# marja-w/gan-des-midi-music-gen

Measured on AMD Instinct MI355X. Metric: GAN training samples/sec (G+D step), higher is better.
Workload: dtype bf16; 1 GPU; SIMNN G/D iteration, synthetic 128x256 spectrogram windows; per_gpu_batch=256, global_batch=256, mode=faithful, parallelism=dp1

## Files before the change

### gan_des_midi_music_gen_amd/csrc/gemm.hip

```cpp
#include "gemm_common.h"

namespace {

constexpr int BM = 64, BN = 64, NT = 256;

template <typename CT> struct GemmCfg;
template <> struct GemmCfg<float> { static constexpr int KT = 32, LD = 34; };
template <> struct GemmCfg<__bf16> { static constexpr int KT = 64, LD = 72; };

template <typename CT, typename TA, typename TB>
__global__ __launch_bounds__(NT) void gemm_kernel(GemmArgs g) {
  constexpr int KT = GemmCfg<CT>::KT, LD = GemmCfg<CT>::LD;
  __shared__ __attribute__((aligned(16))) CT smem[(BM + BN) * LD];
  CT* As = smem;
  CT* Bs = smem + BM * LD;
  const int t = threadIdx.x, l = t & 63, w = t >> 6, wm = w >> 1, wn = w & 1;
  const int lr = l & 15, lg = l >> 4;
  const int m0 = blockIdx.y * BM, n0 = blockIdx.x * BN;
  const int kbeg = blockIdx.z * g.k_per_split;
  const int kend = min(g.K, kbeg + g.k_per_split);
  const TA* __restrict__ A = (const TA*)g.A;
  const TB* __restrict__ B = (const TB*)g.B;
  const bool a_kfast = (g.sak == 1), b_kfast = (g.sbk == 1);
  f32x4 acc[2][2];
#pragma unroll
  for (int i = 0; i < 2; ++i)
#pragma unroll
    for (int j = 0; j < 2; ++j) acc[i][j] = (f32x4){0.f, 0.f, 0.f, 0.f};

  constexpr int PER = BM * KT / NT;
  float va[PER], vb[PER];
  auto load_tile = [&](int k0) {
#pragma unroll
    for (int i = 0; i < PER; ++i) {
      const int idx = t + NT * i;
      const int m = a_kfast ? idx / KT : idx % BM;
      const int k = a_kfast ? idx % KT : idx / BM;
      const int gm = m0 + m, gk = k0 + k;
      va[i] = (gm < g.M && gk < kend) ? to_f32(A[(int64_t)gm * g.sam + (int64_t)gk * g.sak]) : 0.f;
    }
#pragma unroll
    for (int i = 0; i < PER; ++i) {
      const int idx = t + NT * i;
      const int n = b_kfast ? idx / KT : idx % BN;
      const int k = b_kfast ? idx % KT : idx / BN;
      const int gn = n0 + n, gk = k0 + k;
      vb[i] = (gn < g.N && gk < kend) ? to_f32(B[(int64_t)gk * g.sbk + (int64_t)gn * g.sbn]) : 0.f;
    }
  };
  if (kbeg < kend) load_tile(kbeg);
  for (int k0 = kbeg; k0 < kend; k0 += KT) {
#pragma unroll
    for (int i = 0; i < PER; ++i) {
      const int idx = t + NT * i;
      const int m = a_kfast ? idx / KT : idx % BM;
      const int k = a_kfast ? idx % KT : idx / BM;
      As[m * LD + k] = from_f32<CT>(va[i]);
      const int n = b_kfast ? idx / KT : idx % BN;
      const int kb = b_kfast ? idx % KT : idx / BN;
      Bs[n * LD + kb] = from_f32<CT>(vb[i]);
    }
    __syncthreads();
    if (k0 + KT < kend) load_tile(k0 + KT);
    if constexpr (sizeof(CT) == 4) {
#pragma unroll
      for (int ks = 0; ks < KT / 4; ++ks) {
        float a[2], b[2];
#pragma unroll
        for (int i = 0; i < 2; ++i) a[i] = As[(wm * 32 + i * 16 + lr) * LD + ks * 4 + lg];
#pragma unroll
        for (int j = 0; j < 2; ++j) b[j] = Bs[(wn * 32 + j * 16 + lr) * LD + ks * 4 + lg];
#pragma unroll
        for (int i = 0; i < 2; ++i)
#pragma unroll
          for (int j = 0; j < 2; ++j) acc[i][j] = mfma16(a[i], b[j], acc[i][j]);
      }
    } else {
#pragma unroll
      for (int ks = 0; ks < KT / 32; ++ks) {
        bf16x8 a[2], b[2];
#pragma unroll
        for (int i = 0; i < 2; ++i) a[i] = *(const bf16x8*)&As[(wm * 32 + i * 16 + lr) * LD + ks * 32 + lg * 8];
#pragma unroll
        for (int j = 0; j < 2; ++j) b[j] = *(const bf16x8*)&Bs[(wn * 32 + j * 16 + lr) * LD + ks * 32 + lg * 8];
#pragma unroll
        for (int i = 0; i < 2; ++i)
#pragma unroll
          for (int j = 0; j < 2; ++j) acc[i][j] = mfma16(a[i], b[j], acc[i][j]);
      }
    }
    __syncthreads();
  }

#pragma unroll
  for (int i = 0; i < 2; ++i)
#pragma unroll
    for (int j = 0; j < 2; ++j)
#pragma unroll
      for (int r = 0; r < 4; ++r) {
        const int m = m0 + wm * 32 + i * 16 + lg * 4 + r;
        const int n = n0 + wn * 32 + j * 16 + lr;
        if (m < g.M && n < g.N) {
          if (g.split_k > 1) g.ws[((int64_t)blockIdx.z * g.M + m) * g.N + n] = acc[i][j][r];
          else gemm_epilogue_store(g, m, n, acc[i][j][r]);
        }
      }
}

template <bool VEC>
__global__ __launch_bounds__(256) void gemm_splitk_reduce(GemmArgs g) {
  const int64_t total = (int64_t)g.M * g.N;
  if constexpr (VEC) {
    __shared__ f32x4 part[4][64];
    const int lane = threadIdx.x & 63, zg = threadIdx.x >> 6;
    const int64_t idx = ((int64_t)blockIdx.x * 64 + lane) * 4;
    const bool live = idx < total;
    const int q4 = (g.split_k + 3) / 4;
    const int z0 = zg * q4, z1 = min(g.split_k, z0 + q4);
    f32x4 s[4];
#pragma unroll
    for (int q = 0; q < 4; ++q) s[q] = (f32x4){0.f, 0.f, 0.f, 0.f};
    if (live) {
      int z = z0;
      for (; z + 3 < z1; z += 4) {
#pragma unroll
        for (int q = 0; q < 4; ++q) s[q] += *(const f32x4*)(g.ws + (int64_t)(z + q) * total + idx);
      }
      for (; z < z1; ++z) s[0] += *(const f32x4*)(g.ws + (int64_t)z * total + idx);
    }
    part[zg][lane] = (s[0] + s[1]) + (s[2] + s[3]);
    __syncthreads();
    if (zg == 0 && live) {
      const f32x4 v = (part[0][lane] + part[1][lane]) + (part[2][lane] + part[3][lane]);
      const int m = (int)(idx / g.N), n = (int)(idx % g.N);
#pragma unroll
      for (int r = 0; r < 4; ++r) gemm_epilogue_store(g, m, n + r, v[r]);
    }
  } else {
    const int64_t idx = (int64_t)blockIdx.x * 256 + threadIdx.x;
    if (idx >= total) return;
    float s[4] = {0.f, 0.f, 0.f, 0.f};
    int z = 0;
    for (; z + 3 < g.split_k; z += 4) {
#pragma unroll
      for (int q = 0; q < 4; ++q) s[q] += g.ws[(int64_t)(z + q) * total + idx];
    }
    for (; z < g.split_k; ++z) s[0] += g.ws[(int64_t)z * total + idx];
    gemm_epilogue_store(g, (int)(idx / g.N), (int)(idx % g.N), (s[0] + s[1]) + (s[2] + s[3]));
  }
}

int launch_splitk_reduce(const GemmArgs& g, hipStream_t s) {
  if (g.split_k > 1) {
    const int64_t total = (int64_t)g.M * g.N;
    if (g.N % 4 == 0) {
      hipLaunchKernelGGL(gemm_splitk_reduce<true>, dim3((unsigned)((total / 4 + 63) / 64)), dim3(256), 0, s, g);
    } else {
      hipLaunchKernelGGL(gemm_splitk_reduce<false>, dim3((unsigned)((total + 255) / 256)), dim3(256), 0, s, g);
    }
    GDM_LAUNCH_OK("gdm_gemm(split-k reduce)");
  }
  return GDM_OK;
}

template <typename CT>
int launch_gemm(const GemmArgs& g, int a_dtype, int b_dtype, hipStream_t s) {
  dim3 grid((g.N + BN - 1) / BN, (g.M + BM - 1) / BM, g.split_k), block(NT);
  if (a_dtype == GDM_F32 && b_dtype == GDM_F32) hipLaunchKernelGGL((gemm_kernel<CT, float, float>), grid, block, 0, s, g);
  else if (a_dtype == GDM_F32) hipLaunchKernelGGL((gemm_kernel<CT, float, __bf16>), grid, block, 0, s, g);
  else if (b_dtype == GDM_F32) hipLaunchKernelGGL((gemm_kernel<CT, __bf16, float>), grid, block, 0, s, g);
  else hipLaunchKernelGGL((gemm_kernel<CT, __bf16, __bf16>), grid, block, 0, s, g);
  GDM_LAUNCH_OK("gdm_gemm");
  return launch_splitk_reduce(g, s);
}

}

extern "C" int gdm_gemm(const void* A, int a_dtype, int64_t sam, int64_t sak, const void* B, int b_dtype, int64_t sbk,
                        int64_t sbn, void* C, int c_dtype, int64_t scm, int64_t scn, int M, int N, int K,
                        const float* bias_n, const float* bias_m, int act, float slope, int compute_dtype, int split_k,
                        void* workspace, size_t workspace_bytes, void* stream) {
  GDM_REQUIRE(A && B && C, "gdm_gemm: null operand");
  GDM_REQUIRE(M > 0 && N > 0 && K > 0, "gdm_gemm: bad dims M=%d N=%d K=%d", M, N, K);
  GDM_REQUIRE(gdm_dtype_ok(a_dtype) && gdm_dtype_ok(b_dtype) && gdm_dtype_ok(c_dtype) && gdm_dtype_ok(compute_dtype),
              "gdm_gemm: bad dtype");
  GDM_REQUIRE(act >= GDM_ACT_NONE && act <= GDM_ACT_SIGMOID, "gdm_gemm: bad activation %d", act);
  GDM_REQUIRE(split_k >= 1 && split_k <= 65535, "gdm_gemm: bad split_k %d", split_k);
  GemmArgs probe{A, sam, sak, B, sbk, sbn, C, c_dtype, scm, scn, M, N, K, bias_n, bias_m, act, slope, 1, K, nullptr};
  const bool fast = compute_dtype == GDM_BF16 && gdm_gemm_bf16_fast_ok(probe, a_dtype, b_dtype);
  const int KT = fast ? GDM_GEMM_FAST_KT : (compute_dtype == GDM_BF16 ? GemmCfg<__bf16>::KT : GemmCfg<float>::KT);
  int tiles = (K + KT - 1) / KT;
  if (split_k > tiles) split_k = tiles;
  int per = (tiles + split_k - 1) / split_k;
  split_k = (tiles + per - 1) / per;
  if (split_k > 1) {
    if (workspace == nullptr || workspace_bytes < (size_t)split_k * M * N * sizeof(float)) {
      gdm_set_error("gdm_gemm: split_k=%d needs %zu workspace bytes, got %zu", split_k,
                    (size_t)split_k * M * N * sizeof(float), workspace_bytes);
      return GDM_EWORKSPACE;
    }
  }
  GemmArgs g{A, sam, sak, B, sbk, sbn, C, c_dtype, scm, scn, M, N, K, bias_n, bias_m, act, slope,
             split_k, per * KT, (float*)workspace};
  hipStream_t s = (hipStream_t)stream;
  if (fast) {
    int rc = gdm_gemm_bf16_fast_launch(g, a_dtype, b_dtype, s);
    if (rc != GDM_OK) return rc;
    return launch_splitk_reduce(g, s);
  }
  return compute_dtype == GDM_BF16 ? launch_gemm<__bf16>(g, a_dtype, b_dtype, s)
                                   : launch_gemm<float>(g, a_dtype, b_dtype, s);
}
```

### gan_des_midi_music_gen_amd/csrc/gemm_bf16.hip

```cpp
#include <cstdlib>
#include <type_traits>
#include "gemm_common.h"

namespace {

constexpr int BM = 128, BN = 128, NT = 256;

using rsrc_t = __amdgpu_buffer_rsrc_t;
constexpr uint32_t BUF_OOB = 0x80000000u;
typedef uint32_t u32x4 __attribute__((ext_vector_type(4)));
__device__ __forceinline__ rsrc_t make_rsrc(const void* p, uint32_t bytes) {
  const uint64_t a = (uint64_t)p;
  const uint32_t lo = __builtin_amdgcn_readfirstlane((uint32_t)a);
  const uint32_t hi = __builtin_amdgcn_readfirstlane((uint32_t)(a >> 32));
  return __builtin_amdgcn_make_buffer_rsrc((void*)(((uint64_t)hi << 32) | lo), 0,
                                           __builtin_amdgcn_readfirstlane(bytes), 0x00020000);
}

__device__ __forceinline__ void wave_lds_sync() {
  __builtin_amdgcn_fence(__ATOMIC_RELEASE, "wavefront");
  __builtin_amdgcn_wave_barrier();
  __builtin_amdgcn_fence(__ATOMIC_ACQUIRE, "wavefront");
}

__device__ __forceinline__ bf16x4 lds_tr16(const __bf16* p) {
  return __builtin_amdgcn_ds_read_tr16_b64_v4bf16((__attribute__((address_space(3))) bf16x4*)p);
}

template <int ACT> __device__ __forceinline__ float act_const(float v, float slope) {
  if constexpr (ACT == GDM_ACT_RELU) return v > 0.f ? v : 0.f;
  else if constexpr (ACT == GDM_ACT_LEAKY) return v > 0.f ? v : v * slope;
  else if constexpr (ACT == GDM_ACT_SIGMOID) return 1.0f / (1.0f + expf(-v));
  else return v;
}

template <int KT> __device__ __forceinline__ int kswz(int row) { return KT == 64 ? ((row >> 1) & 7) : ((row >> 1) & 2); }
__device__ __forceinline__ int rswz(int k) { return (k & 3) | ((k >> 1) & 4); }

template <typename T, int KT> struct Stage {
  static constexpr int N = 128 * KT * (int)sizeof(T) / 16 / NT;
  f32x4 v[N];
};

template <typename T, int KT> struct Lane {
  uint32_t off[Stage<T, KT>::N];
  int kl[Stage<T, KT>::N];
  int lds[Stage<T, KT>::N];
};

template <typename T, int KT, bool KMAJ>
__device__ __forceinline__ void lane_init(Lane<T, KT>& ln, int64_t ld, int rows, int r0) {
  constexpr int EPC = 16 / sizeof(T);
  const int t = threadIdx.x;
#pragma unroll
  for (int i = 0; i < Stage<T, KT>::N; ++i) {
    const int c = t + NT * i;
    int rl, kl;
    if constexpr (KMAJ) {
      constexpr int CPR = KT / EPC;
      rl = c / CPR; kl = (c % CPR) * EPC;
      ln.off[i] = (uint32_t)(((int64_t)(r0 + rl) * ld + kl) * (int64_t)sizeof(T));
      ln.lds[i] = rl * KT + 8 * ((kl >> 3) ^ kswz<KT>(rl)) + (kl & 7);
    } else {
      constexpr int CPK = 128 / EPC;
      kl = c / CPK; rl = (c % CPK) * EPC;
      ln.off[i] = (uint32_t)(((int64_t)kl * ld + r0 + rl) * (int64_t)sizeof(T));
      ln.lds[i] = kl * 128 + (rl ^ (16 * rswz(kl)));
    }
    ln.kl[i] = (r0 + rl < rows) ? kl : -1;
  }
}

template <typename T, int KT, bool KMAJ>
__device__ __forceinline__ void stage_load(Stage<T, KT>& st, const Lane<T, KT>& ln, rsrc_t rs, int64_t ld, int k0,
                                           int kend) {
  const uint32_t kbytes = (uint32_t)((KMAJ ? (int64_t)k0 : (int64_t)k0 * ld) * (int64_t)sizeof(T));
#pragma unroll
  for (int i = 0; i < Stage<T, KT>::N; ++i) {
    const bool ok = ln.kl[i] >= 0 && k0 + ln.kl[i] < kend;
    st.v[i] = __builtin_bit_cast(f32x4, __builtin_amdgcn_raw_buffer_load_b128(rs, ok ? kbytes + ln.off[i] : BUF_OOB, 0, 0));
  }
}

template <typename T, int KT>
__device__ __forceinline__ void stage_store(const Stage<T, KT>& st, const Lane<T, KT>& ln, __bf16* __restrict__ img) {
#pragma unroll
  for (int i = 0; i < Stage<T, KT>::N; ++i) {
    if constexpr (sizeof(T) == 2) {
      *(f32x4*)(img + ln.lds[i]) = st.v[i];
    } else {
      bf16x4 h;
#pragma unroll
      for (int e = 0; e < 4; ++e) h[e] = (__bf16)st.v[i][e];
      *(bf16x4*)(img + ln.lds[i]) = h;
    }
  }
}

template <int KT, bool KMAJ>
__device__ __forceinline__ bf16x8 frag_read(const __bf16* __restrict__ img, int row0, int kk, int lr, int lg) {
  if constexpr (KMAJ) {
    const int row = row0 + lr;
    return *(const bf16x8*)&img[row * KT + 8 * ((4 * kk + lg) ^ kswz<KT>(row))];
  } else {
    const int q = lr >> 2, p = lr & 3;
    const int kr = 32 * kk + 8 * lg + q;
    const int n = (row0 + 4 * p) ^ (16 * (q | (4 * (lg & 1))));
    const bf16x4 lo = lds_tr16(&img[kr * 128 + n]);
    const bf16x4 hi = lds_tr16(&img[(kr + 4) * 128 + n]);
    return __builtin_shufflevector(lo, hi, 0, 1, 2, 3, 4, 5, 6, 7);
  }
}

template <typename TA, bool A_KMAJ, typename TB, bool B_KMAJ, int KT, int DEPTH>
__global__ __launch_bounds__(NT) void gemm_bf16_fast(GemmArgs g) {
  constexpr int IMG = 128 * KT;
  __shared__ __attribute__((aligned(16))) __bf16 smem[2 * DEPTH * IMG];
  const int t = threadIdx.x, l = t & 63, w = t >> 6, wm = w >> 1, wn = w & 1;
  const int lr = l & 15, lg = l >> 4;
  const int MT = (g.M + BM - 1) / BM, NTl = (g.N + BN - 1) / BN;
  const int id = blockIdx.x;
  const int grp = id / (8 * MT), within = id % (8 * MT);
  const int outer = grp * 8 + (within & 7), mt = within >> 3;
  if (outer >= NTl * g.split_k) return;
  const int nt = outer % NTl, zs = outer / NTl;
  const int m0 = mt * BM, n0 = nt * BN;
  const int kstep = KT * g.split_k;
  const int kbeg = zs * KT;
  const int kend = g.K;
  const int64_t lda = A_KMAJ ? g.sam : g.sak;
  const int64_t ldb = B_KMAJ ? g.sbn : g.sbk;
  const rsrc_t ra = make_rsrc(g.A, (uint32_t)((A_KMAJ ? (int64_t)(g.M - 1) * lda + g.K : (int64_t)(g.K - 1) * lda + g.M) *
                                             (int64_t)sizeof(TA)));
  const rsrc_t rb = make_rsrc(g.B, (uint32_t)((B_KMAJ ? (int64_t)(g.N - 1) * ldb + g.K : (int64_t)(g.K - 1) * ldb + g.N) *
                                             (int64_t)sizeof(TB)));
  Lane<TA, KT> la;
  Lane<TB, KT> lb;
  lane_init<TA, KT, A_KMAJ>(la, lda, g.M, m0);
  lane_init<TB, KT, B_KMAJ>(lb, ldb, g.N, n0);

  f32x4 acc[4][4];
#pragma unroll
  for (int i = 0; i < 4; ++i)
#pragma unroll
    for (int j = 0; j < 4; ++j) acc[i][j] = (f32x4){0.f, 0.f, 0.f, 0.f};

  auto multiply = [&](const __bf16* As, const __bf16* Bs) {
#pragma unroll
    for (int kk = 0; kk < KT / 32; ++kk) {
      bf16x8 a[4], b[4];
#pragma unroll
      for (int i = 0; i < 4; ++i) a[i] = frag_read<KT, A_KMAJ>(As, wm * 64 + 16 * i, kk, lr, lg);
#pragma unroll
      for (int j = 0; j < 4; ++j) b[j] = frag_read<KT, B_KMAJ>(Bs, wn * 64 + 16 * j, kk, lr, lg);
#pragma unroll
      for (int i = 0; i < 4; ++i)
#pragma unroll
        for (int j = 0; j < 4; ++j) acc[i][j] = mfma16(b[j], a[i], acc[i][j]);
    }
  };
  Stage<TA, KT> sa[DEPTH];
  Stage<TB, KT> sb[DEPTH];
  if constexpr (DEPTH == 2) {
    auto tile = [&](Stage<TA, KT>& xa, Stage<TB, KT>& xb, __bf16* As, int k0) {
      __bf16* Bs = As + IMG;
      stage_store<TA, KT>(xa, la, As);
      stage_store<TB, KT>(xb, lb, Bs);
      __syncthreads();
      stage_load<TA, KT, A_KMAJ>(xa, la, ra, lda, k0 + 2 * kstep, kend);
      stage_load<TB, KT, B_KMAJ>(xb, lb, rb, ldb, k0 + 2 * kstep, kend);
      multiply(As, Bs);
    };
    stage_load<TA, KT, A_KMAJ>(sa[0], la, ra, lda, kbeg, kend);
    stage_load<TB, KT, B_KMAJ>(sb[0], lb, rb, ldb, kbeg, kend);
    stage_load<TA, KT, A_KMAJ>(sa[1], la, ra, lda, kbeg + kstep, kend);
    stage_load<TB, KT, B_KMAJ>(sb[1], lb, rb, ldb, kbeg + kstep, kend);
    for (int k0 = kbeg; k0 < kend; k0 += 2 * kstep) {
      tile(sa[0], sb[0], smem, k0);
      tile(sa[DEPTH - 1], sb[DEPTH - 1], smem + 2 * IMG * (DEPTH - 1), k0 + kstep);
    }
  } else {
    __bf16* As = smem;
    __bf16* Bs = smem + IMG;
    stage_load<TA, KT, A_KMAJ>(sa[0], la, ra, lda, kbeg, kend);
    stage_load<TB, KT, B_KMAJ>(sb[0], lb, rb, ldb, kbeg, kend);
    for (int k0 = kbeg; k0 < kend; k0 += kstep) {
      __syncthreads();
      stage_store<TA, KT>(sa[0], la, As);
      stage_store<TB, KT>(sb[0], lb, Bs);
      __syncthreads();
      stage_load<TA, KT, A_KMAJ>(sa[0], la, ra, lda, k0 + kstep, kend);
      stage_load<TB, KT, B_KMAJ>(sb[0], lb, rb, ldb, k0 + kstep, kend);
      multiply(As, Bs);
    }
  }

  auto epilogue = [&](auto act_tag) {
    constexpr int ACT = decltype(act_tag)::value;
    const bool vec_ok = (g.N % 4 == 0);
    if (g.split_k > 1) {
#pragma unroll
      for (int i = 0; i < 4; ++i) {
        const int m = m0 + wm * 64 + 16 * i + lr;
        if (m >= g.M) continue;
#pragma unroll
        for (int j = 0; j < 4; ++j) {
          const int n = n0 + wn * 64 + 16 * j + 4 * lg;
          if (n >= g.N) continue;
          float* dst = g.ws + ((int64_t)zs * g.M + m) * g.N + n;
#ifndef GDM_GEMM_DEFAULT_STORES
          if (vec_ok) __builtin_nontemporal_store(acc[i][j], (f32x4*)dst);
#else
          if (vec_ok) *(f32x4*)dst = acc[i][j];
#endif
          else
            for (int r = 0; r < 4 && n + r < g.N; ++r) dst[r] = acc[i][j][r];
        }
      }
      return;
    }
    if (vec_ok && m0 + BM <= g.M && n0 + BN <= g.N &&
        (g.c_dtype != GDM_BF16 || (g.scm % 8 == 0 && ((uintptr_t)g.C & 15) == 0))) {
      __syncthreads();
      float* scr = (float*)smem + w * (16 * 64);
      const bool is_bf16 = g.c_dtype == GDM_BF16;
      const int prow = is_bf16 ? (l >> 3) : (l >> 4), pcol = is_bf16 ? 8 * (l & 7) : 4 * (l & 15);
      const int nn = n0 + wn * 64 + pcol;
      f32x4 bn0 = {0.f, 0.f, 0.f, 0.f}, bn1 = bn0;
      if (g.bias_n) {
        bn0 = *(const f32x4*)(g.bias_n + nn);
        if (is_bf16) bn1 = *(const f32x4*)(g.bias_n + nn + 4);
      }
      const bool has_bias = g.bias_n || g.bias_m;
#pragma unroll
      for (int i = 0; i < 4; ++i) {
        wave_lds_sync();
#pragma unroll
        for (int j = 0; j < 4; ++j) *(f32x4*)&scr[lr * 64 + 4 * ((4 * j + lg) ^ lr)] = acc[i][j];
        wave_lds_sync();
        if (is_bf16) {
#pragma unroll
          for (int h = 0; h < 2; ++h) {
            const int row = 8 * h + prow, c8 = l & 7;
            f32x4 v0 = *(const f32x4*)&scr[row * 64 + 4 * ((2 * c8) ^ row)];
            f32x4 v1 = *(const f32x4*)&scr[row * 64 + 4 * ((2 * c8 + 1) ^ row)];
            const int m = m0 + wm * 64 + 16 * i + row;
            if (has_bias) {
              const float bm = g.bias_m ? g.bias_m[m] : 0.f;
              v0 += bn0 + (f32x4){bm, bm, bm, bm};
              v1 += bn1 + (f32x4){bm, bm, bm, bm};
            }
            bf16x8 hv;
#pragma unroll
            for (int r = 0; r < 4; ++r) {
              hv[r] = (__bf16)act_const<ACT>(v0[r], g.slope);
              hv[4 + r] = (__bf16)act_const<ACT>(v1[r], g.slope);
            }
#ifndef GDM_GEMM_DEFAULT_STORES
            __builtin_nontemporal_store(hv, (bf16x8*)((__bf16*)g.C + (int64_t)m * g.scm + nn));
#else
            *(bf16x8*)((__bf16*)g.C + (int64_t)m * g.scm + nn) = hv;
#endif
          }
        } else {
#pragma unroll
          for (int h = 0; h < 4; ++h) {
            const int row = 4 * h + prow, pc = l & 15;
            f32x4 v = *(const f32x4*)&scr[row * 64 + 4 * (pc ^ row)];
            const int m = m0 + wm * 64 + 16 * i + row;
            if (has_bias) {
              const float bm = g.bias_m ? g.bias_m[m] : 0.f;
              v += bn0 + (f32x4){bm, bm, bm, bm};
            }
#pragma unroll
            for (int r = 0; r < 4; ++r) v[r] = act_const<ACT>(v[r], g.slope);
#ifndef GDM_GEMM_DEFAULT_STORES
            __builtin_nontemporal_store(v, (f32x4*)((float*)g.C + (int64_t)m * g.scm + nn));
#else
            *(f32x4*)((float*)g.C + (int64_t)m * g.scm + nn) = v;
#endif
          }
        }
      }
      return;
    }
#pragma unroll
    for (int i = 0; i < 4; ++i) {
      const int m = m0 + wm * 64 + 16 * i + lr;
      if (m >= g.M) continue;
#pragma unroll
      for (int j = 0; j < 4; ++j) {
        const int n = n0 + wn * 64 + 16 * j + 4 * lg;
        if (n >= g.N) continue;
        f32x4 v = acc[i][j];
        for (int r = 0; r < 4 && n + r < g.N; ++r) {
          float y = v[r];
          if (g.bias_n) y += g.bias_n[n + r];
          if (g.bias_m) y += g.bias_m[m];
          store_from_f32(g.C, g.c_dtype, (int64_t)m * g.scm + n + r, act_const<ACT>(y, g.slope));
        }
      }
    }
  };
  switch (g.act) {
    case GDM_ACT_RELU: epilogue(std::integral_constant<int, GDM_ACT_RELU>{}); break;
    case GDM_ACT_LEAKY: epilogue(std::integral_constant<int, GDM_ACT_LEAKY>{}); break;
    case GDM_ACT_SIGMOID: epilogue(std::integral_constant<int, GDM_ACT_SIGMOID>{}); break;
    default: epilogue(std::integral_constant<int, GDM_ACT_NONE>{}); break;
  }
}

template <typename TA, bool AK, typename TB, bool BK>
void launch_v(const GemmArgs& g, int variant, dim3 grid, hipStream_t s) {
  if (variant == 1) hipLaunchKernelGGL((gemm_bf16_fast<TA, AK, TB, BK, 64, 2>), grid, dim3(NT), 0, s, g);
  else hipLaunchKernelGGL((gemm_bf16_fast<TA, AK, TB, BK, 32, 1>), grid, dim3(NT), 0, s, g);
}
template <typename TA, bool AK, typename TB>
void launch_b(const GemmArgs& g, bool b_kmaj, int variant, dim3 grid, hipStream_t s) {
  if (b_kmaj) launch_v<TA, AK, TB, true>(g, variant, grid, s);
  else launch_v<TA, AK, TB, false>(g, variant, grid, s);
}
template <typename TA, bool AK>
void launch_a(const GemmArgs& g, int b_dtype, bool b_kmaj, int variant, dim3 grid, hipStream_t s) {
  if (b_dtype == GDM_BF16) launch_b<TA, AK, __bf16>(g, b_kmaj, variant, grid, s);
  else launch_b<TA, AK, float>(g, b_kmaj, variant, grid, s);
}

inline bool operand_ok(const void* p, int dtype, int64_t s_row, int64_t s_k, int rows, int K, bool* kmaj) {
  const int64_t esz = dtype == GDM_BF16 ? 2 : 4, epc = 16 / esz;
  if (((uintptr_t)p & 15) != 0) return false;
  if (s_k == 1 && s_row >= 1 && (s_row * esz) % 16 == 0 && K % epc == 0) {
    *kmaj = true;
    return ((int64_t)(rows - 1) * s_row + K) * esz < ((int64_t)1 << 31);
  }
  if (s_row == 1 && s_k >= 1 && (s_k * esz) % 16 == 0 && rows % epc == 0) {
    *kmaj = false;
    return ((int64_t)(K - 1) * s_k + rows) * esz < ((int64_t)1 << 31);
  }
  return false;
}

}

bool gdm_gemm_bf16_fast_ok(const GemmArgs& g, int a_dtype, int b_dtype) {
  bool ak, bk;
  if (!operand_ok(g.A, a_dtype, g.sam, g.sak, g.M, g.K, &ak)) return false;
  if (!operand_ok(g.B, b_dtype, g.sbn, g.sbk, g.N, g.K, &bk)) return false;
  if (g.scn != 1) return false;
  const int64_t csz = g.c_dtype == GDM_BF16 ? 2 : 4;
  if (g.N % 4 == 0) {
    if ((g.scm * csz) % (4 * csz) != 0 || ((uintptr_t)g.C & (4 * csz - 1)) != 0) return false;
    if (g.bias_n && ((uintptr_t)g.bias_n & 15) != 0) return false;
  }
  if ((int64_t)g.M * g.N < 64 * 64) return false;
  return true;
}

int gdm_gemm_bf16_fast_launch(const GemmArgs& g, int a_dtype, int b_dtype, hipStream_t s) {
  bool ak = true, bk = true;
  operand_ok(g.A, a_dtype, g.sam, g.sak, g.M, g.K, &ak);
  operand_ok(g.B, b_dtype, g.sbn, g.sbk, g.N, g.K, &bk);
  const int MT = (g.M + BM - 1) / BM, NTl = (g.N + BN - 1) / BN;
  const int outer = NTl * g.split_k;
  dim3 grid((unsigned)(((outer + 7) / 8) * 8 * MT));
  int variant = (g.split_k > 1 && (int64_t)outer * MT <= 512 && g.k_per_split >= 256) ? 1 : 0;
  static const char* force = getenv("GDM_GEMM_VARIANT");
  if (force && force[0]) variant = force[0] == '1';
  if (a_dtype == GDM_BF16) {
    if (ak) launch_a<__bf16, true>(g, b_dtype, bk, variant, grid, s); else launch_a<__bf16, false>(g, b_dtype, bk, variant, grid, s);
  } else {
    if (ak) launch_a<float, true>(g, b_dtype, bk, variant, grid, s); else launch_a<float, false>(g, b_dtype, bk, variant, grid, s);
  }
  GDM_LAUNCH_OK("gdm_gemm(bf16 fast path)");
  return GDM_OK;
}
```

Before: 428,300 samples/s.

## Add persistent streaming GEMM kernel for fc1 input-gradient with K=128

Adds a specialized persistent kernel for bf16 GEMMs with K=128, small M (128-512) and very large N, such as the fc1 dX backward. It keeps the whole A operand in registers per wave and streams B tiles through LDS with double-buffered register prefetch. Output is staged through swizzled LDS scratch so it can be written with vectorized nontemporal stores. A 16-way unrolled load path is also added to the split-K reduce to raise memory-level parallelism. The cost is more kernel specialization and higher register pressure.

```diff
diff --git a/gan_des_midi_music_gen_amd/csrc/gemm.hip b/gan_des_midi_music_gen_amd/csrc/gemm.hip
--- a/gan_des_midi_music_gen_amd/csrc/gemm.hip
+++ b/gan_des_midi_music_gen_amd/csrc/gemm.hip
@@ -122,6 +122,13 @@
     for (int q = 0; q < 4; ++q) s[q] = (f32x4){0.f, 0.f, 0.f, 0.f};
     if (live) {
       int z = z0;
+      for (; z + 15 < z1; z += 16) {
+        f32x4 v[16];
+#pragma unroll
+        for (int i = 0; i < 16; ++i) v[i] = *(const f32x4*)(g.ws + (int64_t)(z + i) * total + idx);
+#pragma unroll
+        for (int i = 0; i < 16; ++i) s[i & 3] += v[i];
+      }
       for (; z + 3 < z1; z += 4) {
 #pragma unroll
         for (int q = 0; q < 4; ++q) s[q] += *(const f32x4*)(g.ws + (int64_t)(z + q) * total + idx);
diff --git a/gan_des_midi_music_gen_amd/csrc/gemm_bf16.hip b/gan_des_midi_music_gen_amd/csrc/gemm_bf16.hip
--- a/gan_des_midi_music_gen_amd/csrc/gemm_bf16.hip
+++ b/gan_des_midi_music_gen_amd/csrc/gemm_bf16.hip
@@ -310,6 +310,114 @@
   }
 }
 
+constexpr int DX_NT = 512, DX_K = 128;
+
+template <int RT>
+__global__ __launch_bounds__(DX_NT) void fc1_dx_stream(GemmArgs g, int ntiles) {
+  __shared__ __attribute__((aligned(16))) __bf16 Bs[DX_K * 128];
+  __shared__ __attribute__((aligned(16))) float scratch[(DX_NT / 64) * 16 * 64];
+  const int t = threadIdx.x, l = t & 63, w = t >> 6, lr = l & 15, lg = l >> 4;
+  const int64_t lda = g.sam, ldb = g.sbk;
+  const rsrc_t ra = make_rsrc(g.A, (uint32_t)(((int64_t)(g.M - 1) * lda + DX_K) * 2));
+  const rsrc_t rb = make_rsrc(g.B, (uint32_t)(((int64_t)(DX_K - 1) * ldb + g.N) * 2));
+  const int mw = w * 16 * RT;
+  const bool wave_live = mw < g.M;
+
+  bf16x8 a[RT][4];
+#pragma unroll
+  for (int i = 0; i < RT; ++i)
+#pragma unroll
+    for (int kk = 0; kk < 4; ++kk) {
+      const int row = mw + 16 * i + lr;
+      const uint32_t off = row < g.M ? (uint32_t)(((int64_t)row * lda + 32 * kk + 8 * lg) * 2) : BUF_OOB;
+      a[i][kk] = __builtin_bit_cast(bf16x8, __builtin_amdgcn_raw_buffer_load_b128(ra, off, 0, 0));
+    }
+
+  uint32_t boff[4];
+  int blds[4];
+#pragma unroll
+  for (int i = 0; i < 4; ++i) {
+    const int c = t + DX_NT * i, kl = c >> 4, rl = (c & 15) * 8;
+    boff[i] = (uint32_t)(((int64_t)kl * ldb + rl) * 2);
+    blds[i] = kl * 128 + (rl ^ (16 * rswz(kl)));
+  }
+  u32x4 st[4];
+  auto load_tile = [&](int tile) {
+    const uint32_t nb = (uint32_t)tile * 256u;
+#pragma unroll
+    for (int i = 0; i < 4; ++i)
+      st[i] = __builtin_amdgcn_raw_buffer_load_b128(rb, tile < ntiles ? nb + boff[i] : BUF_OOB, 0, 0);
+  };
+
+  float* scr = scratch + w * (16 * 64);
+  const int prow = l >> 3, c8 = l & 7;
+  load_tile(blockIdx.x);
+  for (int tile = blockIdx.x; tile < ntiles; tile += gridDim.x) {
+    __syncthreads();
+#pragma unroll
+    for (int i = 0; i < 4; ++i) *(u32x4*)(Bs + blds[i]) = st[i];
+    __syncthreads();
+    load_tile(tile + gridDim.x);
+    if (!wave_live) continue;
+    const int n0 = tile * 128;
+#pragma unroll
+    for (int h = 0; h < 2; ++h) {
+      bf16x8 b[4][4];
+#pragma unroll
+      for (int j = 0; j < 4; ++j)
+#pragma unroll
+        for (int kk = 0; kk < 4; ++kk) b[j][kk] = frag_read<32, false>(Bs, 64 * h + 16 * j, kk, lr, lg);
+#pragma unroll
+      for (int i = 0; i < RT; ++i) {
+        f32x4 acc[4];
+#pragma unroll
+        for (int j = 0; j < 4; ++j) acc[j] = (f32x4){0.f, 0.f, 0.f, 0.f};
+#pragma unroll
+        for (int kk = 0; kk < 4; ++kk)
+#pragma unroll
+          for (int j = 0; j < 4; ++j) acc[j] = mfma16(b[j][kk], a[i][kk], acc[j]);
+        wave_lds_sync();
+#pragma unroll
+        for (int j = 0; j < 4; ++j) *(f32x4*)&scr[lr * 64 + 4 * ((4 * j + lg) ^ lr)] = acc[j];
+        wave_lds_sync();
+#pragma unroll
+        for (int hh = 0; hh < 2; ++hh) {
+          const int row = 8 * hh + prow;
+          const f32x4 v0 = *(const f32x4*)&scr[row * 64 + 4 * ((2 * c8) ^ row)];
+          const f32x4 v1 = *(const f32x4*)&scr[row * 64 + 4 * ((2 * c8 + 1) ^ row)];
+          bf16x8 hv;
+#pragma unroll
+          for (int r = 0; r < 4; ++r) {
+            hv[r] = (__bf16)v0[r];
+            hv[4 + r] = (__bf16)v1[r];
+          }
+          const int m = mw + 16 * i + row;
+          if (m < g.M)
+            __builtin_nontemporal_store(hv, (bf16x8*)((__bf16*)g.C + (int64_t)m * g.scm + n0 + 64 * h + 8 * c8));
+        }
+      }
+    }
+  }
+}
+
+inline int dx_stream_grid(int ntiles) {
+  static int cus = 0;
+  if (cus == 0) {
+    int dev = 0, n = 256;
+    if (hipGetDevice(&dev) != hipSuccess || hipDeviceGetAttribute(&n, hipDeviceAttributeMultiprocessorCount, dev) != hipSuccess)
+      n = 256;
+    cus = n > 0 ? n : 256;
+  }
+  const int rounds = (ntiles + cus - 1) / cus;
+  return (ntiles + rounds - 1) / rounds;
+}
+
+inline bool dx_stream_ok(const GemmArgs& g, int a_dtype, int b_dtype, bool ak, bool bk) {
+  return a_dtype == GDM_BF16 && b_dtype == GDM_BF16 && g.c_dtype == GDM_BF16 && ak && !bk && g.K == DX_K &&
+         g.split_k == 1 && g.M > 128 && g.M <= 512 && g.N >= 8192 && g.N % 128 == 0 && !g.bias_n && !g.bias_m &&
+         g.act == GDM_ACT_NONE && g.scm % 8 == 0 && ((uintptr_t)g.C & 15) == 0;
+}
+
 template <typename TA, bool AK, typename TB, bool BK>
 void launch_v(const GemmArgs& g, int variant, dim3 grid, hipStream_t s) {
   if (variant == 1) hipLaunchKernelGGL((gemm_bf16_fast<TA, AK, TB, BK, 64, 2>), grid, dim3(NT), 0, s, g);
@@ -360,6 +468,14 @@
   bool ak = true, bk = true;
   operand_ok(g.A, a_dtype, g.sam, g.sak, g.M, g.K, &ak);
   operand_ok(g.B, b_dtype, g.sbn, g.sbk, g.N, g.K, &bk);
+  if (dx_stream_ok(g, a_dtype, b_dtype, ak, bk)) {
+    const int ntiles = g.N / 128;
+    const dim3 sgrid((unsigned)dx_stream_grid(ntiles));
+    if (g.M > 256) hipLaunchKernelGGL(fc1_dx_stream<4>, sgrid, dim3(DX_NT), 0, s, g, ntiles);
+    else hipLaunchKernelGGL(fc1_dx_stream<2>, sgrid, dim3(DX_NT), 0, s, g, ntiles);
+    GDM_LAUNCH_OK("gdm_gemm(fc1 dX stream)");
+    return GDM_OK;
+  }
   const int MT = (g.M + BM - 1) / BM, NTl = (g.N + BN - 1) / BN;
   const int outer = NTl * g.split_k;
   dim3 grid((unsigned)(((outer + 7) / 8) * 8 * MT));
```

Result: faster. 433,500 samples/s (median of 6 runs) (+1.2%).
